# blyssprivacy/sdk

Hardware: AMD Instinct MI355X
Metric: PIR queries/sec (full answer path) on 2^20 items x 256 B (higher is better)
Workload: dtype u64; 1 GPU; spiral-rs process_query, c2 = {"db_item_size": 256, "instances": 1, "n": 2, "nu_1": 9, "nu_2": 11, "p": 256, "q2_bits": 20, "t_conv": 4, "t_exp_left": 8, "t_exp_right": 56, "t_gsw": 8}, encoded DB 64.0 GiB (56.0 GiB resident per GPU), unsharded, one query per step

## Files before the change

sdk_amd/csrc/bodies.hpp:

```cpp
#pragma once
#include "device_common.hpp"

namespace spiral {

__device__ __forceinline__ void ntt_fwd_body(const DevTables& T, const FwdDesc& d, int o, int c, u32* ldsA, u32* ldsB) {
  const int tau = threadIdx.x;
  const int rows = d.rdim * d.t;
  const int per_b = rows * d.cols;
  const int b = o / per_b;
  const int rem = o - b * per_b;
  const int row = rem / d.cols, col = rem - row * d.cols;
  const int kdig = row / d.rdim, j = row - kdig * d.rdim;
  long sb = d.src_idx ? (long)d.src_idx[b] : (long)b;
  if (d.delta_off) sb = (long)(b / d.delta_inner) * d.delta_outer_stride + (b % d.delta_inner);
  const u64* src = d.src + (sb * d.src_batch_stride + (long)(d.src_row0 + j) * d.src_cols + col) * N;
  const ModConst m = T.c.mod[c];
  const int sh = kdig * d.bits;
  const bool plain = (d.bits >= 64);
  const u64 mask = plain ? ~0ULL : ((1ULL << d.bits) - 1ULL);
  u32 v[8];
#pragma unroll
  for (int k = 0; k < 8; k++) {
    u64 x = src[tau + 256 * k];
    u64 piece = (sh >= 64) ? 0ULL : ((x >> sh) & mask);
// ... 45 lines not shown
  if (d.scal) {
    if (p >= d.n_polys) {
      const int e = p - d.n_polys;
      const int ct = d.scal_only_idx[e >> 1], r = e & 1;
      const long sp = ((long)(ct - d.scal_thresh) * 2 + r) * 2 * N, dp = ((long)ct * 2 + r) * 2 * N;
#pragma unroll
      for (int c = 0; c < 2; c++) {
        const uint4* a = reinterpret_cast<const uint4*>(d.src + sp + c * N + 8 * tau);
        const uint4* b = reinterpret_cast<const uint4*>(d.scal + c * N + 8 * tau);
        const uint4 a0 = a[0], a1 = a[1], b0 = b[0], b1 = b[1];
        const ModConst m = T.c.mod[c];
        uint4* o = reinterpret_cast<uint4*>(d.scal_dst + dp + c * N + 8 * tau);
        o[0] = make_uint4(reduce64((u64)a0.x * b0.x, m), reduce64((u64)a0.y * b0.y, m), reduce64((u64)a0.z * b0.z, m), reduce64((u64)a0.w * b0.w, m));
        o[1] = make_uint4(reduce64((u64)a1.x * b1.x, m), reduce64((u64)a1.y * b1.y, m), reduce64((u64)a1.z * b1.z, m), reduce64((u64)a1.w * b1.w, m));
      }
      return;
    }
    const int e = p / d.polys_per_idx, r = p - e * d.polys_per_idx;
    const int ct = d.idx[e];
    if (ct >= d.scal_thresh) {
      scal_store = base;
      base = (long)(ct - d.scal_thresh) * d.idx_stride + (long)r * d.poly_stride;
    }
  }
  u32 res[2][8];
#pragma unroll
  for (int c = 0; c < 2; c++) {
    const ModConst m = T.c.mod[c];
    const u32* src = d.src + base + (long)c * crt_stride;
    u32 v[8];
    if (z_stride == 1 && ((base | crt_stride | (scal_store < 0 ? 0 : scal_store)) & 3) == 0) {
      const uint4 a0 = reinterpret_cast<const uint4*>(src + 8 * tau)[0], a1 = reinterpret_cast<const uint4*>(src + 8 * tau)[1];
      v[0] = a0.x; v[1] = a0.y; v[2] = a0.z; v[3] = a0.w; v[4] = a1.x; v[5] = a1.y; v[6] = a1.z; v[7] = a1.w;
      if (d.premod) {
#pragma unroll
        for (int k = 0; k < 8; k++) v[k] %= m.q;
      }
      if (scal_store >= 0) {
        const uint4 s0 = reinterpret_cast<const uint4*>(d.scal + c * N + 8 * tau)[0], s1 = reinterpret_cast<const uint4*>(d.scal + c * N + 8 * tau)[1];
        const u32 sc[8] = {s0.x, s0.y, s0.z, s0.w, s1.x, s1.y, s1.z, s1.w};
#pragma unroll
        for (int k = 0; k < 8; k++) v[k] = reduce64((u64)v[k] * (u64)sc[k], m);
        uint4* o = reinterpret_cast<uint4*>(d.scal_dst + scal_store + (long)c * crt_stride + 8 * tau);
        o[0] = make_uint4(v[0], v[1], v[2], v[3]);
        o[1] = make_uint4(v[4], v[5], v[6], v[7]);
      }
// ... 216 lines not shown
```

sdk_amd/csrc/capi.cpp:

```cpp
#include <cstdlib>
#include <new>

#include "capi_internal.hpp"

using namespace spiral;

static thread_local std::string g_last_error;
static thread_local int g_last_rc = SP_OK;
static thread_local int g_shard_split_hint = 1;
int spiral::guarded_status(int rc, const char* what) {
  if (rc != SP_OK) g_last_error = what;
  g_last_rc = rc;
  return rc;
}
int spiral::null_handle_rc() { return g_last_rc != SP_OK ? g_last_rc : SP_E_ARG; }

void spiral::check_device(int dev) {
  int cur = 0;
  HIP_CHECK(hipGetDevice(&cur));
  if (cur != dev) throw ArgError("handle belongs to HIP device " + std::to_string(dev) + " but the current device is " + std::to_string(cur));
}

void spiral::download_ntt(Workspace& W, const u32* src, size_t words, uint64_t* host, DevBuf<u64>& tmp) {
  tmp.ensure(words);
// ... 611 lines not shown
  if (!name) return SP_E_ARG;
  set_tunable(name, value);
  return SP_OK;
}
extern "C" void sp_shard_split_hint_(int on) { g_shard_split_hint = on; }
extern "C" int sp_scatter_group_choice_(const sp_db_t* db, int G) {
  if (db && db->sparse) {
    tunables_new_call();
    return db->col_G == 1 && db->num_shards == G && sparse_group_min() != 0 ? SPARSE_GROUP_MAX : 1;
  }
  if (db && db->planar_resident) return db->num_shards == G && G > 1 ? planar_resident_group_max(db->nj) : 1;
  if (!db || !db->packed || db->col_G != 1 || db->num_shards != G) return 1;
  SweepBatchDesc d{};
  d.batch = SWEEP_BATCH_MAX;
  d.num_per = db->np_local;
  d.nj = db->nj;
  tunables_new_call();
  return sweep_batch_scatter_ok(d, G) && G <= (int)tunable("batch_scatter_max_g", BATCH_SCATTER_MAX_G_DEFAULT) ? SWEEP_BATCH_MAX : 1;
}
extern "C" int sp_shard_group_max_(const sp_db_t* db) {
  return db && db->planar_resident && db->num_shards > 1 ? planar_resident_group_max(db->nj) : SWEEP_BATCH_MAX;
}
extern "C" int sp_db_num_shards_(const sp_db_t* db) { return db ? db->num_shards : 0; }
void sp_set_last_error_(const char* msg) { g_last_error = msg ? msg : ""; }
void sp_note_path_(uint64_t bits) { note_path(bits); }

const char* sp_path_name(int bit) {
  static const char* names[] = {"sweep_packed_persist", "sweep_packed", "sweep_wide", "sweep_narrow", "sweep_batch",
                                "from_sweep4", "from_sweep1", "fold_fused", "fold_tail_delta", "fold_tail_literal",
                                "pipelined_fold_overlap", "expand_pruned", "pack_v1", "direct_upload", "scatter_out",
                                "from_sweep4_xcd_order", "fold_tail_persistent", "expand_round_one_launch", "sweep_sparse",
                                "rccl_in_library", "fold_wave", "cu_split_overlap", "expand_split", "pipe_class_split",
                                "sweep_batch_mfma", "custom_transport", "from_sweep_wave",
                                "fold_tail_batched", "sweep_ring", "sweep_batch_mfma_two_tiles", "fold_wave8", "sweep_batch_planar",
                                "expand_group", "expand_wave", "sweep_batch_scatter", "sparse_group_pass", "sweep_narrow_group"};
  return bit >= 0 && bit < (int)(sizeof(names) / sizeof(names[0])) ? names[bit] : nullptr;
}

int sp_device_count(void) {
  int n = 0;
  if (hipGetDeviceCount(&n) != hipSuccess) {
    (void)hipGetLastError();
    return 0;
  }
  return n;
}
// ... 811 lines not shown
```

sdk_amd/csrc/fold.hip:

```cpp
#include <type_traits>

#include "device_common.hpp"
#include "wave_ntt.hpp"
#include "bodies.hpp"

namespace spiral {

__device__ __forceinline__ bool fold_zero_shortcut(const u64* ct0, const u64* ct1, u64* out, int tau) {
  int nz0 = 0, nz1 = 0;
#pragma unroll
  for (int k = 0; k < 16; k++) {
    nz0 |= ct0[tau + 256 * k] != 0;
    nz1 |= ct1[tau + 256 * k] != 0;
  }
  const int any0 = __syncthreads_or(nz0), any1 = __syncthreads_or(nz1);
  if (any0 && any1) return false;
  const u64* src = any0 ? ct0 : ct1;
#pragma unroll
  for (int k = 0; k < 16; k++) out[tau + 256 * k] = src[tau + 256 * k];
  return true;
}

__global__ __launch_bounds__(256, 2) void k_fold_fused(DevTables T, FoldDesc d) {
  __shared__ u32 lds0[LDS_WORDS];
// ... 451 lines not shown

__global__ __launch_bounds__(256, 2) void k_expand_wave(DevTables T, ExpandWaveDesc d, GroupOff g) {
  extern __shared__ __attribute__((aligned(16))) u32 smem_fw[];
  u32* wbuf = smem_fw;
  u32* ltw = smem_fw + 4 * WBUF_WORDS;
  u64* raw0 = reinterpret_cast<u64*>(ltw + 2 * N);
  const int tau = threadIdx.x, lane = tau & 63;
  const int wv = __builtin_amdgcn_readfirstlane(tau >> 6);
  const int b = (int)blockIdx.x, c = (int)blockIdx.y, qi = (int)blockIdx.z;
  const ModConst m = T.c.mod[c];
  const u32* fw = T.tw + (size_t)c * 4 * N;
  const u64* src = group_rebase(d.raw, g.raw[qi]) + (size_t)d.pos[b] * 2 * N;
  const u32* A_w = group_rebase(d.A_w, g.pp[qi]);
  u32* vout = group_rebase(d.v, g.v[qi]);
  u32* mybuf = wbuf + wv * WBUF_WORDS;
  wtw_stage(ltw, wave_fwd_image(T.tw, c), tau);
#pragma unroll
  for (int k = 0; k < 8; k++) raw0[tau + 256 * k] = src[tau + 256 * k];
  __syncthreads();
  const u64 mask = (1ULL << d.bits) - 1ULL;
  u64 acc0[32], acc1[32];
#pragma unroll
  for (int k = 0; k < 32; k++) acc0[k] = acc1[k] = 0;
#pragma unroll 1
  for (int dg = wv; dg <= d.t; dg += 4) {
    int ln = lane;
    const u32* fwi = fw;
    asm volatile("" : "+v"(ln));
    asm volatile("" : "+s"(fwi));
    WaveScalarTw stw;
    wntt_scalar_tw(stw, fwi);
    u32 v[32];
    if (dg < d.t) {
      const int sh = dg * d.bits;
#pragma unroll
      for (int k = 0; k < 32; k++) v[k] = sh < 64 ? (u32)((raw0[64 * k + ln] >> (sh & 63)) & mask) : 0u;
    } else {
#pragma unroll
      for (int k = 0; k < 32; k++) v[k] = reduce64(src[(size_t)N + 64 * k + ln], m);
    }
    SP_SB();
    const u32* a0 = dg < d.t ? A_w + ((size_t)dg * 2 + c) * N : d.const_w;
    const u32* a1 = dg < d.t ? A_w + ((size_t)(d.t + dg) * 2 + c) * N : d.const_w + N;
    FoldMac hk{acc0, acc1, reinterpret_cast<const u32x4w_t*>(a0) + ln, reinterpret_cast<const u32x4w_t*>(a1) + ln};
    wntt_fwd<false>(v, ln, mybuf, fwi, stw, ltw, m.q, m.two_q, hk);
  }
  int lt = lane;
  asm volatile("" : "+v"(lt));
// ... 12 lines not shown
}
#define SP_ADD(R, REGION)                                                                              \
_Pragma("unroll") for (int g4 = 0; g4 < 8; g4++) {                                                   \
  const u32x4w_t t4 = sc[(REGION) * 512 + g4 * 64 + lt];                                             \
  R[4 * g4] = add_mod(R[4 * g4], t4.x, m.q); R[4 * g4 + 1] = add_mod(R[4 * g4 + 1], t4.y, m.q);      \
  R[4 * g4 + 2] = add_mod(R[4 * g4 + 2], t4.z, m.q); R[4 * g4 + 3] = add_mod(R[4 * g4 + 3], t4.w, m.q); \
}
  __syncthreads();
  if (wv == 2) { SP_PUT(r0, 0) SP_PUT(r1, 1) }
  if (wv == 3) { SP_PUT(r0, 2) SP_PUT(r1, 3) }
  __syncthreads();
  if (wv == 0) { SP_ADD(r0, 0) SP_ADD(r0, 2) }
  if (wv == 1) { SP_ADD(r1, 1) SP_ADD(r1, 3) }
  __syncthreads();
  if (wv == 0) { SP_PUT(r1, 0) }
  if (wv == 1) { SP_PUT(r0, 1) }
  __syncthreads();
  if (wv == 0) { SP_ADD(r0, 1) }
  if (wv == 1) { SP_ADD(r1, 0) }
#undef SP_PUT
#undef SP_ADD
  if (wv < 2) {
    u32* o = vout + ((size_t)d.out_idx[b] * 2 + c) * N + (size_t)wv * 2 * N + 32 * lt;
#pragma unroll
    for (int g4 = 0; g4 < 8; g4++) {
      const uint4 a = reinterpret_cast<const uint4*>(o)[g4];
      uint4 w;
      w.x = add_mod(wv == 0 ? r0[4 * g4] : r1[4 * g4], a.x, m.q);
      w.y = add_mod(wv == 0 ? r0[4 * g4 + 1] : r1[4 * g4 + 1], a.y, m.q);
      w.z = add_mod(wv == 0 ? r0[4 * g4 + 2] : r1[4 * g4 + 2], a.z, m.q);
      w.w = add_mod(wv == 0 ? r0[4 * g4 + 3] : r1[4 * g4 + 3], a.w, m.q);
      reinterpret_cast<uint4*>(o)[g4] = w;
    }
  }
}
void launch_expand_wave(const DevTables& T, const ExpandWaveDesc& d, const GroupOff& g, int B, hipStream_t s) {
  if (d.cnt <= 0 || B <= 0) return;
  const size_t lds = (size_t)(4 * WBUF_WORDS + 2 * N) * 4 + (size_t)N * 8;
  hipLaunchKernelGGL(k_expand_wave, dim3(d.cnt, 2, B), dim3(256), lds, s, T, d, g);
  launched(PATH_EXPAND_FUSED | PATH_EXPAND_WAVE, "k_expand_wave");
}

__global__ __launch_bounds__(256) void k_mats_to_wave(MatsToWaveDesc d) { mats_to_wave_body(d, blockIdx.x); }
void launch_mats_to_wave(u32* dst, const u32* src, size_t n_words, hipStream_t s, int half_polys) {
  if (n_words == 0) return;
  const MatsToWaveDesc d{dst, src, n_words, half_polys};
  hipLaunchKernelGGL(k_mats_to_wave, dim3((unsigned)((n_words + 255) / 256)), dim3(256), 0, s, d);
  launched(0, "k_mats_to_wave");
}
// ... 42 lines not shown
```

sdk_amd/csrc/kernels.hpp:

```cpp
#pragma once
#include <hip/hip_runtime.h>

#include <vector>

#include "params.hpp"

namespace spiral {

constexpr int N = (int)POLY_LEN;

struct DevTables {
  const u32* tw;
  DevConsts c;
};
__host__ __device__ inline const u32* inv_tables(const u32* tw, int c) { return tw + (size_t)8 * N + (size_t)c * 2 * N; }
__host__ __device__ inline const u32* wave_fwd_image(const u32* tw, int c) { return tw + (size_t)12 * N + (size_t)c * 2 * N; }
__host__ __device__ inline int wtw_phys(int idx) {
  if (idx >= 1024) {
    const int L = (idx - 1024) >> 4, r = (idx - 1024) & 15;
    return 1024 + 16 * L + 4 * (((r >> 2) + (L >> 2)) & 3) + (r & 3);
  }
  if (idx >= 512) {
    const int L = (idx - 512) >> 3, r = (idx - 512) & 7;
    return 512 + 8 * L + 4 * (((r >> 2) + (L >> 3)) & 1) + (r & 3);
// ... 61 lines not shown
};
void launch_ntt_fwd(const DevTables& T, const FwdDesc& d, hipStream_t s);
void launch_ntt_fwd3(const DevTables& T, const FwdDesc& d0, const FwdDesc& d1, const FwdDesc& d2, hipStream_t s);

float bench_ntt_core(const DevTables& T, int M, int blocks, int reps, u32* scratch, hipStream_t s);

struct InvDesc {
  const u32* src;
  const int* idx;
  int polys_per_idx;
  long idx_stride, poly_stride, crt_stride, z_stride;
  u64* dst;
  int n_polys;
  int premod;
  int sweep_np;
  int automorph_t;
  const u32* scal;
  u32* scal_dst;
  int scal_thresh;
  const int* scal_only_idx;
  int n_scalar_only;
  const u64* addend;
  int add_inner2, add_outer_stride;
};
void launch_ntt_inv(const DevTables& T, const InvDesc& d, hipStream_t s);
void launch_from_sweep4(const DevTables& T, const u32* src, int np, int n_planes, int premod, u64* dst, hipStream_t s);

struct MacDesc {
  const u32* A;
  const u32* B;
  u32* out;
  const u32* addend;
  const int* out_idx;
  int R, K;
  int A_row_stride;
  int batch_inner, batch_outer;
  long B_inner_stride, B_outer_stride;
  int split_k;
  long split_off;
  int out_batch_stride, out_row_stride;
  const u32* extra;
  const int* extra_idx;
  int extra_row;
};
void launch_mac(const DevTables& T, const MacDesc& d, hipStream_t s);
void launch_mac2(const DevTables& T, const MacDesc& d0, const MacDesc& d1, hipStream_t s);

struct ExpandSideDesc {
  const u64* raw;
  const int* pos;
  const int* out_idx;
  const u32* A;
  u32* v;
  int cnt, t, bits;
};
void launch_expand_round(const DevTables& T, const ExpandSideDesc& left, const ExpandSideDesc& right, hipStream_t s);
constexpr long EXPAND_ROUND_MIN_DEFAULT = 2048;

constexpr int GROUP_MAX = 16;
struct GroupOff {
  long long v[GROUP_MAX], raw[GROUP_MAX], dig[GROUP_MAX], ct1[GROUP_MAX], pp[GROUP_MAX];
};
void launch_ntt_inv_group(const DevTables& T, const InvDesc& d, const GroupOff& g, int B, hipStream_t s);
void launch_ntt_fwd3_group(const DevTables& T, const FwdDesc& d0, const FwdDesc& d1, const FwdDesc& d2, const GroupOff& g, int B,
                           hipStream_t s);
void launch_mac2_group(const DevTables& T, const MacDesc& d0, const MacDesc& d1, const GroupOff& g, int B, hipStream_t s);
void launch_expand_round_group(const DevTables& T, const ExpandSideDesc& left, const ExpandSideDesc& right, const GroupOff& g, int B,
                               hipStream_t s);
void launch_reorient_group(u64* out, const u32* v, int first, int step, int dim0, const GroupOff& g, int B, hipStream_t s);
void launch_copy_polys_group(u32* dst, const int* dst_idx, int dst_row_stride, const u32* src, const int* src_idx, int src_row_stride,
                             int R, int batch, const GroupOff& g, int B, hipStream_t s);
void launch_folding_neg_group(const DevTables& T, u32* mats, const u32* gadget_ntt, int nu2, int two_t, const GroupOff& g, int B,
                              hipStream_t s);
void launch_mats_to_wave_group(u32* dst, const u32* src, size_t n_words, int half_polys, const GroupOff& g, int B, hipStream_t s);
struct ExpandWaveDesc {
  const u64* raw;
  const int* pos;
  const int* out_idx;
  const u32* A_w;
  const u32* const_w;
  u32* v;
  int cnt, t, bits;
};
void launch_expand_wave(const DevTables& T, const ExpandWaveDesc& d, const GroupOff& g, int B, hipStream_t s);
constexpr long EXPAND_WAVE_MIN_DIGITS_DEFAULT = 16;
constexpr long EXPAND_GROUP_ROUND_MIN_DEFAULT = 4096;

struct FoldDesc {
  const u64* X;
  u64* Y;
  const u32* mats;
  int cur, half, planes;
  int t, bits;
  int t_live;
  int zero_shortcuts;
  const u32* mats_w;
};
void launch_mats_to_wave(u32* dst, const u32* src, size_t n_words, hipStream_t s, int half_polys = 0);
constexpr long FOLD_VARIANT_DEFAULT = 5;
void launch_fold_fused(const DevTables& T, const FoldDesc& d, hipStream_t s);

void launch_add_poly_into(const DevTables& T, u32* dst, const int* idx, const u32* src, int batch, hipStream_t s);
void launch_scalar_mul(const DevTables& T, u32* base, long dst_off, long src_off, const u32* scalar, int n_polys,
                       hipStream_t s);
void launch_add_polys_idx(const DevTables& T, u32* dst, const int* di, const u32* a, const int* ai, const u32* b,
// ... 249 lines not shown
```

sdk_amd/csrc/ntt.hip:

```cpp
#include "device_common.hpp"
#include "bodies.hpp"

namespace spiral {

template <int M>
__global__ __launch_bounds__(256) void k_ntt_core_bench(DevTables T, u32* out, int reps) {
  __shared__ u32 lds0[M * LDS_WORDS];
  __shared__ u32 lds1[M * LDS_WORDS];
  const int tau = threadIdx.x;
  const ModConst m = T.c.mod[blockIdx.x & 1];
  const u32* fw = T.tw + (size_t)(blockIdx.x & 1) * 4 * N;
  u32 v[M][8];
#pragma unroll
  for (int mm = 0; mm < M; mm++)
#pragma unroll
    for (int k = 0; k < 8; k++) v[mm][k] = (tau * 2654435761u + k * 40503u + mm + blockIdx.x) % m.q;
  u32* la = lds0;
  u32* lb = lds1;
  for (int r = 0; r < reps; r++) {
    const u32* fwk = fw;
    int tk = tau;
    asm volatile("" : "+s"(fwk));
    asm volatile("" : "+v"(tk));
    ntt_fwd_block_m<M>(v, tk, la, lb, fwk, fwk + N, m.q, m.two_q);
// ... 126 lines not shown
#pragma unroll
    for (int mm = 0; mm < GD; mm++) {
      const int kk = k0 + mm;
      if (kk < d.t) {
        const uint4* a0 = reinterpret_cast<const uint4*>(d.A + ((size_t)kk * 2 + c) * N + 8 * tk);
        const uint4* a1 = reinterpret_cast<const uint4*>(d.A + ((size_t)(d.t + kk) * 2 + c) * N + 8 * tk);
        const uint4 p0 = a0[0], p1 = a0[1], r0 = a1[0], r1 = a1[1];
        acc0[0] += (u64)p0.x * v[mm][0]; acc0[1] += (u64)p0.y * v[mm][1]; acc0[2] += (u64)p0.z * v[mm][2]; acc0[3] += (u64)p0.w * v[mm][3];
        acc0[4] += (u64)p1.x * v[mm][4]; acc0[5] += (u64)p1.y * v[mm][5]; acc0[6] += (u64)p1.z * v[mm][6]; acc0[7] += (u64)p1.w * v[mm][7];
        acc1[0] += (u64)r0.x * v[mm][0]; acc1[1] += (u64)r0.y * v[mm][1]; acc1[2] += (u64)r0.z * v[mm][2]; acc1[3] += (u64)r0.w * v[mm][3];
        acc1[4] += (u64)r1.x * v[mm][4]; acc1[5] += (u64)r1.y * v[mm][5]; acc1[6] += (u64)r1.z * v[mm][6]; acc1[7] += (u64)r1.w * v[mm][7];
      }
    }
    if (((k0 / GD) & 7) == 7) {
#pragma unroll
      for (int k = 0; k < 8; k++) {
        acc0[k] = reduce64(acc0[k], m);
        acc1[k] = reduce64(acc1[k], m);
      }
    }
    __syncthreads();
  }
  u32 e1[8];
#pragma unroll
  for (int k = 0; k < 8; k++) e1[k] = reduce64(src[(size_t)N + tau + 256 * k], m);
  ntt_fwd_block(e1, tau, lds0, lds1, fw, fw + N, m.q, m.two_q);
  u32* o0 = d.v + ((size_t)d.out_idx[b] * 2 + c) * N + 8 * tau;
  u32* o1 = o0 + (size_t)2 * N;
  const uint4 g0 = reinterpret_cast<const uint4*>(o0)[0], g1 = reinterpret_cast<const uint4*>(o0)[1];
  const uint4 h0 = reinterpret_cast<const uint4*>(o1)[0], h1 = reinterpret_cast<const uint4*>(o1)[1];
  const u32 ga[8] = {g0.x, g0.y, g0.z, g0.w, g1.x, g1.y, g1.z, g1.w};
  const u32 ha[8] = {h0.x, h0.y, h0.z, h0.w, h1.x, h1.y, h1.z, h1.w};
  u32 w0[8], w1[8];
#pragma unroll
  for (int k = 0; k < 8; k++) {
    w0[k] = reduce64(acc0[k] + ga[k], m);
    w1[k] = reduce64(acc1[k] + (u64)ha[k] + e1[k], m);
  }
  reinterpret_cast<uint4*>(o0)[0] = make_uint4(w0[0], w0[1], w0[2], w0[3]);
  reinterpret_cast<uint4*>(o0)[1] = make_uint4(w0[4], w0[5], w0[6], w0[7]);
  reinterpret_cast<uint4*>(o1)[0] = make_uint4(w1[0], w1[1], w1[2], w1[3]);
  reinterpret_cast<uint4*>(o1)[1] = make_uint4(w1[4], w1[5], w1[6], w1[7]);
}
__global__ __launch_bounds__(256) void k_expand_round(DevTables T, ExpandSideDesc dl, ExpandSideDesc dr) {
  __shared__ u32 lds0[EXPAND_GD * LDS_WORDS];
  __shared__ u32 lds1[EXPAND_GD * LDS_WORDS];
  const bool right = (int)blockIdx.x >= dl.cnt;
  expand_round_body(T, right ? dr : dl, (int)blockIdx.x - (right ? dl.cnt : 0), blockIdx.y, lds0, lds1);
}
__global__ __launch_bounds__(256) void k_expand_round_group(DevTables T, ExpandSideDesc dl, ExpandSideDesc dr, GroupOff g) {
  __shared__ u32 lds0[EXPAND_GD * LDS_WORDS];
  __shared__ u32 lds1[EXPAND_GD * LDS_WORDS];
  const int qi = blockIdx.z;
  const bool right = (int)blockIdx.x < dr.cnt;
  ExpandSideDesc d = right ? dr : dl;
  d.raw = group_rebase(d.raw, g.raw[qi]);
  d.A = group_rebase(d.A, g.pp[qi]);
  d.v = group_rebase(d.v, g.v[qi]);
  expand_round_body(T, d, (int)blockIdx.x - (right ? 0 : dr.cnt), blockIdx.y, lds0, lds1);
}
void launch_expand_round_group(const DevTables& T, const ExpandSideDesc& left, const ExpandSideDesc& right, const GroupOff& g, int B,
                               hipStream_t s) {
  const int total = std::max(left.cnt, 0) + std::max(right.cnt, 0);
  if (total <= 0 || B <= 0) return;
  ExpandSideDesc a = left, b = right;
  a.cnt = std::max(a.cnt, 0);
  b.cnt = std::max(b.cnt, 0);
  hipLaunchKernelGGL(k_expand_round_group, dim3(total, 2, B), dim3(256), 0, s, T, a, b, g);
  launched(PATH_EXPAND_FUSED | PATH_EXPAND_GROUP, "k_expand_round_group");
}
void launch_expand_round(const DevTables& T, const ExpandSideDesc& left, const ExpandSideDesc& right, hipStream_t s) {
  const int total = std::max(left.cnt, 0) + std::max(right.cnt, 0);
  if (total <= 0) return;
  ExpandSideDesc a = left, b = right;
  a.cnt = std::max(a.cnt, 0);
  b.cnt = std::max(b.cnt, 0);
  hipLaunchKernelGGL(k_expand_round, dim3(total, 2), dim3(256), 0, s, T, a, b);
  launched(PATH_EXPAND_FUSED, "k_expand_round");
}

__global__ __launch_bounds__(256) void k_ntt_inv(DevTables T, InvDesc d) {
  __shared__ u32 ldsA[LDS_WORDS];
  __shared__ u32 ldsB[LDS_WORDS];
  ntt_inv_body(T, d, blockIdx.x, ldsA, ldsB);
}
__global__ __launch_bounds__(256) void k_ntt_inv_group(DevTables T, InvDesc d, GroupOff g) {
  __shared__ u32 ldsA[LDS_WORDS];
  __shared__ u32 ldsB[LDS_WORDS];
  const int qi = blockIdx.y;
  d.src = group_rebase(d.src, g.v[qi]);
  d.scal_dst = group_rebase(d.scal_dst, g.v[qi]);
  d.dst = group_rebase(d.dst, g.raw[qi]);
  ntt_inv_body(T, d, blockIdx.x, ldsA, ldsB);
}
void launch_ntt_inv_group(const DevTables& T, const InvDesc& d, const GroupOff& g, int B, hipStream_t s) {
  const int blocks = d.n_polys + (d.scal ? 2 * d.n_scalar_only : 0);
  if (blocks <= 0 || B <= 0) return;
  hipLaunchKernelGGL(k_ntt_inv_group, dim3(blocks, B), dim3(256), 0, s, T, d, g);
  launched(PATH_EXPAND_GROUP, "k_ntt_inv_group");
}
void launch_ntt_inv(const DevTables& T, const InvDesc& d, hipStream_t s) {
  const int blocks = d.n_polys + (d.scal ? 2 * d.n_scalar_only : 0);
  if (blocks <= 0) return;
  hipLaunchKernelGGL(k_ntt_inv, dim3(blocks), dim3(256), 0, s, T, d);
  launched(d.sweep_np > 0 ? PATH_FROM_SWEEP1 : 0, "k_ntt_inv");
}

__global__ __launch_bounds__(256, 2) void k_from_sweep4(DevTables T, const u32* src, int np, int premod, u64* dst, int xcd_map) {
  __shared__ u32 lds0[4 * LDS_WORDS];
  __shared__ u32 lds1[4 * LDS_WORDS];
  const int tau = threadIdx.x;
  int g = blockIdx.x;
  if (xcd_map & 1) {
    const int xcd = g & 7, t = g >> 3;
    g = ((t >> 3) * 8 + xcd) * 8 + (t & 7);
// ... 64 lines not shown
```

sdk_amd/csrc/params.cpp:

```cpp
#include "params.hpp"
#include "kernels.hpp"

#include <cctype>
#include <cmath>
#include <map>
#include <stdexcept>

namespace spiral {

typedef unsigned __int128 u128;

u64 mul_mod(u64 a, u64 b, u64 m) { return (u64)((u128)a * b % m); }
u64 pow_mod(u64 a, u64 e, u64 m) {
  u64 r = 1 % m;
  a %= m;
  while (e) {
    if (e & 1) r = mul_mod(r, a, m);
    a = mul_mod(a, a, m);
    e >>= 1;
  }
  return r;
}
u64 inv_mod(u64 a, u64 m) {
  __int128 t = 0, nt = 1, r = m, nr = a % m;
// ... 102 lines not shown
      u64 half = (ipw & 1) ? (ipw + q) >> 1 : ipw >> 1;
      fw[idx] = (u32)pw;
      fwp[idx] = (u32)((pw << 32) / q);
      iw[idx] = (u32)half;
      iwp[idx] = (u32)((half << 32) / q);
      const u64 lz = idx < 2 ? mul_mod(ipw, n_inv, q) : ipw;
      lw[idx] = (u32)lz;
      lwp[idx] = (u32)((lz << 32) / q);
      pw = mul_mod(pw, psi, q);
      ipw = mul_mod(ipw, psi_inv, q);
    }
    if (poly_len == (size_t)N) {
      u32* img = ntt_tables.data() + (size_t)CRT_COUNT * 6 * poly_len + (size_t)c * 2 * poly_len;
      for (size_t i = 0; i < poly_len; i++) {
        const int ph = wtw_phys((int)i);
        img[ph] = 0u - fw[i];
        img[poly_len + ph] = fwp[i];
      }
    }
    dc.mod[c].q = (u32)q;
    dc.mod[c].two_q = (u32)(2 * q);
    dc.mod[c].m64 = (u64)((((u128)1) << 64) / q);
  }
  dc.Q = modulus;
  u64 inv = inv_mod(moduli[0] % moduli[1], moduli[1]);
  dc.q0_inv_q1 = (u32)inv;
  dc.q0_inv_q1_sh = (u32)((inv << 32) / moduli[1]);
}

static std::map<std::string, double> parse_flat_json(const std::string& s) {
  std::map<std::string, double> out;
  size_t i = 0, n = s.size();
  auto skip = [&]() {
    while (i < n && isspace((unsigned char)s[i])) i++;
  };
  skip();
  if (i >= n || s[i] != '{') throw std::runtime_error("params json: expected '{'");
  i++;
  for (;;) {
    skip();
    if (i < n && s[i] == '}') break;
    if (i >= n || (s[i] != '"' && s[i] != '\'')) throw std::runtime_error("params json: expected key");
    char qc = s[i++];
    size_t k0 = i;
    while (i < n && s[i] != qc) i++;
    if (i >= n) throw std::runtime_error("params json: unterminated key");
// ... 89 lines not shown
```

sdk_amd/csrc/params.hpp:

```cpp
#pragma once
static_assert(__BYTE_ORDER__ == __ORDER_LITTLE_ENDIAN__, "spiral_hip assumes a little-endian host");
#include <cstddef>
#include <cstdint>
#include <string>
#include <vector>

namespace spiral {

typedef uint64_t u64;
typedef uint32_t u32;

constexpr size_t POLY_LEN = 2048;
constexpr size_t POLY_LEN_LOG2 = 11;
constexpr size_t CRT_COUNT = 2;
constexpr u64 MODULUS_0 = 268369921ULL;
constexpr u64 MODULUS_1 = 249561089ULL;
constexpr size_t SEED_LENGTH = 32;

struct ModConst {
  u32 q;
  u32 two_q;
  u64 m64;
};

struct DevConsts {
  ModConst mod[2];
  u64 Q;
  u32 q0_inv_q1;
  u32 q0_inv_q1_sh;
};

struct Params {
  size_t poly_len = POLY_LEN, poly_len_log2 = POLY_LEN_LOG2, crt_count = CRT_COUNT;
  u64 moduli[2] = {MODULUS_0, MODULUS_1};
  u64 modulus = 0, modulus_log2 = 0;
  double noise_width = 6.4;
  size_t n = 0;
  u64 pt_modulus = 0, q2_bits = 0;
  size_t t_conv = 0, t_exp_left = 0, t_exp_right = 0, t_gsw = 0;
  bool expand_queries = true;
  size_t db_dim_1 = 0, db_dim_2 = 0, instances = 1, db_item_size = 0, version = 0;
  std::vector<u32> ntt_tables;
  DevConsts dc;

  size_t dim0() const { return (size_t)1 << db_dim_1; }
  size_t num_per() const { return (size_t)1 << db_dim_2; }
  size_t num_items() const { return dim0() * num_per(); }
  size_t trials() const { return n * n; }
  size_t planes() const { return instances * n * n; }
  size_t g() const;
  size_t stop_round() const;
  size_t setup_bytes() const;
  size_t query_bytes() const;
  size_t response_bytes() const;
  size_t db_words() const { return planes() * num_items() * poly_len; }
  bool has_expansion_right_on_wire() const { return version == 0 || t_exp_right != t_exp_left; }
  size_t bits_per(size_t dim) const;
  u64 q2() const;
  const u32* table(int crt, int which) const { return ntt_tables.data() + ((size_t)crt * 4 + which) * poly_len; }

  static Params from_json(const std::string& json);
  void finish();
};

u64 mul_mod(u64 a, u64 b, u64 m);
u64 pow_mod(u64 a, u64 e, u64 m);
// ... 4 lines not shown
```

sdk_amd/csrc/pipeline.hpp:

```cpp
#pragma once
#include <vector>

#include "server.hpp"

namespace spiral {

struct Workspace {
  const Params* P;
  DeviceState* D;
  int device = -1;
  hipStream_t stream = nullptr;
  hipStream_t stream2 = nullptr;
  std::vector<hipEvent_t> ev_plane;
  hipEvent_t ev_fold = nullptr;
  hipEvent_t ev_round0 = nullptr, ev_right = nullptr;
  bool right_pending = false;
  bool long_sweep_follows = false;
  hipEvent_t ev_sw[2] = {nullptr, nullptr};
  bool have_sweep_span = false;
  bool pipelined = false;
  hipEvent_t ev[5] = {nullptr, nullptr, nullptr, nullptr, nullptr};
  DevBuf<u64> q_raw;
  DevBuf<u32> v;
  DevBuf<u64> exp_raw;
// ... 19 lines not shown
  DevBuf<u64> group_q_raw;
  u64* h_packed = nullptr;
  size_t h_packed_words = 0;
  DevBuf<u64> enc_out;
  uint8_t* h_response = nullptr;
  bool host_pinned = true;
  int out_G = 1;
  bool zero_shortcuts = false;
  long fused_min_pairs = 256;

  Workspace(const Params& P, DeviceState& D);
  ~Workspace();
  Workspace(const Workspace&) = delete;
  Workspace& operator=(const Workspace&) = delete;
  void ensure_expand();
  void ensure_sweep();
  void ensure_finish();
  size_t plane_group() const;
};

void run_coefficient_expansion(Workspace& W, const sp_pp& pp, size_t g_rounds, const DeviceState::PrunedPlan* plan = nullptr,
                               int tree = 0, size_t r_begin = 0);
void join_right(Workspace& W);
void run_regev_to_gsw(Workspace& W, const sp_pp& pp, const u32* v_src, const int* src_ct, const int* src_poly);
void run_folding_neg(Workspace& W);
void run_mats_to_wave(Workspace& W, size_t levels, bool c_only = false);
void run_fold_operands(Workspace& W);
void run_begin_direct(Workspace& W, const uint8_t* query);
void run_begin_group(Workspace* const* Ws, const sp_pp* const* pps, const uint8_t* const* queries, const size_t* query_lens, int B);
void run_begin(Workspace& W, const sp_pp& pp, const uint8_t* query, size_t query_len, int j0 = 0, int nj = 0,
               const DeviceState::PrunedPlan* plan = nullptr);
void run_sweep_sparse(Workspace& W, const sp_db& db, const int* col_ptr, const int* col_rows, const int* col_slots);
void run_sweep_sparse_group(Workspace* const* Ws, int B, const sp_db& db, const int* col_ptr, const int* col_rows, const int* col_slots,
                            hipStream_t s);
void run_sweep_sparse_scatter(Workspace& W, const sp_db& db, const int* col_ptr, const int* col_rows, const int* col_slots, int G,
                              int plane0, int n_planes, bool per_plane);
void run_sweep_sparse_scatter_group(Workspace* const* Ws, int B, const sp_db& db, const int* col_ptr, const int* col_rows,
                                    const int* col_slots, int G, hipStream_t s);
std::unique_ptr<DeviceState::PrunedPlan> build_pruned_plan_rows(const Params& P, const std::vector<char>& rows);
void run_sweep(Workspace& W, const sp_db& db);
void run_sweep_pipelined(Workspace& W, const sp_db& db);
bool sweep_is_pipelined(const Params& p, const sp_db& db);
void launch_plane_sweep(Workspace& W, const sp_db& db, size_t plane);
bool fused_fold_supported(const Params& p);
struct FoldOpts {
  long fused_min_pairs;
// ... 16 lines not shown
```

sdk_amd/csrc/server.cpp:

```cpp
#include "server.hpp"

#include <algorithm>
#include <atomic>
#include <cstdlib>
#include <cstring>
#include <functional>

#include "pipeline.hpp"

namespace spiral {

void hip_check(hipError_t e, const char* what, const char* file, int line) {
  if (e != hipSuccess) {
    (void)hipGetLastError();
    throw HipError(std::string(what) + " failed at " + file + ":" + std::to_string(line) + ": " + hipGetErrorString(e));
  }
}

static std::mutex g_tun_mu;
static std::vector<std::pair<std::string, long>> g_tun;
static std::atomic<unsigned> g_tun_epoch{1};
static std::atomic<long> g_fresh_allocs{0};
void tunables_new_call() { g_tun_epoch.fetch_add(1, std::memory_order_relaxed); }
void set_tunable(const char* name, long v) {
// ... 343 lines not shown

std::unique_ptr<DeviceState::PrunedPlan> build_pruned_plan_rows(const Params& P, const std::vector<char>& rows) {
  auto pl = std::make_unique<DeviceState::PrunedPlan>();
  pl->j0 = -1;
  pl->nj = -1;
  std::vector<int> L;
  pl->rounds = build_round_plans(P, 0, 0, L, &rows);
  pl->rounds_even = build_round_plans(P, 0, 0, L, &rows, 1);
  pl->rounds_odd = build_round_plans(P, 0, 0, L, &rows, 2);
  pl->lists.alloc(std::max<size_t>(L.size(), 1));
  if (!L.empty()) upload_words(pl->lists.p, L.data(), L.size() * sizeof(int));
  return pl;
}

static std::unique_ptr<DeviceState> build_device_state(const Params& P, int device) {
  auto D = std::make_unique<DeviceState>();
  D->device = device;
  D->tw.alloc(P.ntt_tables.size());
  upload_words(D->tw.p, P.ntt_tables.data(), P.ntt_tables.size() * sizeof(u32));
  D->T.tw = D->tw.p;
  D->T.c = P.dc;
  const size_t g = P.expand_queries ? P.g() : 0;
  const size_t nu2 = P.db_dim_2;

  {
    std::vector<u64> raw(std::max<size_t>(g, 1) * POLY_LEN, 0);
    for (size_t r = 0; r < g && r < POLY_LEN_LOG2; r++) raw[r * POLY_LEN + (POLY_LEN - ((size_t)1 << r))] = P.modulus - 1;
    DevBuf<u64> d_raw(raw.size());
    h2d_sync(d_raw.p, raw.data(), raw.size() * 8);
    D->neg1.alloc(std::max<size_t>(g, 1) * 2 * POLY_LEN);
    FwdDesc f{d_raw.p, nullptr, D->neg1.p, (int)g, 1, 1, 1, 64, 1, 0, 1};
    launch_ntt_fwd(D->T, f, 0);
    HIP_CHECK(hipDeviceSynchronize());
  }
  {
    const size_t cols = 2 * P.t_gsw, bits = P.bits_per(P.t_gsw);
    std::vector<u64> raw(2 * cols * POLY_LEN, 0);
    for (size_t i = 0; i < 2; i++)
      for (size_t j = 0; j < P.t_gsw; j++) {
        if (bits * j >= 64) continue;
        raw[(i * cols + (i + j * 2)) * POLY_LEN] = 1ULL << (bits * j);
      }
    DevBuf<u64> d_raw(raw.size());
    h2d_sync(d_raw.p, raw.data(), raw.size() * 8);
    D->gadget_gsw.alloc(2 * cols * 2 * POLY_LEN);
    FwdDesc f{d_raw.p, nullptr, D->gadget_gsw.p, (int)(2 * cols), 1, 1, 1, 64, 1, 0, 1};
// ... 252 lines not shown
  const Params& p = *W.P;
  DeviceState& D = *W.D;
  u64* const exp_raw = tree == 2 ? W.exp_raw_r.p : W.exp_raw.p;
  u32* const exp_dig = tree == 2 ? W.exp_dig_r.p : W.exp_dig.p;
  u32* const exp_ct1 = tree == 2 ? W.exp_ct1_r.p : W.exp_ct1.p;
  const int tl = (int)p.t_exp_left, tr = (int)p.t_exp_right;
  RoundLaunches R{};
  InvDesc& inv = R.inv;
  inv.src = W.v.p;
  inv.idx = L + rp.all_ct;
  inv.polys_per_idx = 2;
  inv.idx_stride = 4 * POLY_LEN;
  inv.poly_stride = 2 * POLY_LEN;
  inv.crt_stride = POLY_LEN;
  inv.z_stride = 1;
  inv.dst = exp_raw;
  inv.n_polys = rp.n_all * 2;
  inv.automorph_t = rp.t_auto;
  inv.scal = D.neg1.p + r * 2 * POLY_LEN;
  inv.scal_dst = W.v.p;
  inv.scal_thresh = rp.num_in;
  inv.scal_only_idx = L + rp.skip2;
  inv.n_scalar_only = rp.n_skip2;
  for (int side = 0; side < 2; side++) {
    const int cnt = side == 0 ? rp.n_left : rp.n_right;
    const int t = side == 0 ? tl : tr;
    FwdDesc f{};
    f.src = exp_raw;
    f.src_idx = L + (side == 0 ? rp.left_pos : rp.right_pos);
    f.dst = exp_dig + (side == 0 ? 0 : (size_t)rp.n_left * tl * 2 * POLY_LEN);
    f.n_out = cnt * t;
    f.rdim = 1;
    f.cols = 1;
    f.t = t;
    f.bits = (int)p.bits_per(t);
    f.src_batch_stride = 2;
    f.src_row0 = 0;
    f.src_cols = 1;
    R.fd[side] = f;
  }
  {
    FwdDesc f1{};
    f1.src = exp_raw;
    f1.dst = exp_ct1;
    f1.n_out = rp.n_all;
    f1.rdim = 1;
    f1.cols = 1;
    f1.t = 1;
    f1.bits = 64;
    f1.src_batch_stride = 2;
    f1.src_row0 = 1;
    f1.src_cols = 1;
    R.fd[2] = f1;
  }
  R.round_transforms = (long)rp.n_left * tl + (long)rp.n_right * tr;
  R.digits_fit = R.fd[0].bits <= 28 && R.fd[1].bits <= 28;
  for (int side = 0; side < 2; side++) {
    const int cnt = side == 0 ? rp.n_left : rp.n_right;
    const int t = side == 0 ? tl : tr;
    const bool use_right = side == 1 && pp.has_right && p.db_dim_2 > 0;
    const size_t woff = use_right ? pp.off_right + r * 2 * tr : pp.off_left + r * 2 * tl;
    MacDesc m{};
    m.A = pp.all.p + woff * 2 * POLY_LEN;
    m.B = R.fd[side].dst;
    m.out = W.v.p;
    m.addend = W.v.p;
    m.out_idx = L + (side == 0 ? rp.left_out : rp.right_out);
    m.R = 2;
    m.K = t;
    m.batch_inner = cnt;
    m.batch_outer = 1;
    m.B_inner_stride = t;
    m.B_outer_stride = 0;
    m.split_k = t;
    m.split_off = 0;
    m.out_batch_stride = 0;
    m.out_row_stride = 1;
    m.extra = exp_ct1;
    m.extra_idx = L + (side == 0 ? rp.left_pos : rp.right_pos);
    m.extra_row = 1;
    R.md[side] = m;
    R.es[side] = ExpandSideDesc{R.fd[side].src, R.fd[side].src_idx, m.out_idx, m.A, m.out, m.batch_inner, R.fd[side].t, R.fd[side].bits};
  }
  return R;
}

void run_coefficient_expansion(Workspace& W, const sp_pp& pp, size_t g_rounds, const DeviceState::PrunedPlan* plan,
                               int tree, size_t r_begin) {
  DeviceState& D = *W.D;
  hipStream_t s = W.stream;
  const int* L = plan ? plan->lists.p : D.lists.p;
  const std::vector<RoundPlan>& rounds = tree == 1   ? (plan ? plan->rounds_even : D.rounds_even)
                                         : tree == 2 ? (plan ? plan->rounds_odd : D.rounds_odd)
                                                     : (plan ? plan->rounds : D.rounds);
  for (size_t r = r_begin; r < g_rounds; r++) {
    const RoundPlan& rp = rounds[r];
    if (rp.n_all == 0 && (tree != 0 || rp.n_skip2 == 0)) continue;
    const RoundLaunches R = round_launches(W, pp, rp, r, L, tree);
    const bool one_launch = R.round_transforms >= tunable("expand_round_min", EXPAND_ROUND_MIN_DEFAULT) && R.digits_fit &&
                            (tree != 2 || tunable("expand_round_odd", 0) != 0);
    launch_ntt_inv(D.T, R.inv, s);
    if (one_launch) {
      launch_expand_round(D.T, R.es[0], R.es[1], s);
    } else {
      launch_ntt_fwd3(D.T, R.fd[0], R.fd[1], R.fd[2], s);
// ... 28 lines not shown
  for (int i = 0; i < B; i++) {
    wave_ok = wave_ok && pps[i]->all_w.p != nullptr && pps[i]->all_w.n == pps[0]->all_w.n;
    if (wave_ok) gw.pp[i] = off(pps[i]->all_w.p, pps[0]->all_w.p);
  }
  for (size_t r = 0; r < g_rounds; r++) {
    const RoundPlan& rp = D.rounds[r];
    if (rp.n_all == 0 && rp.n_skip2 == 0) continue;
    const RoundLaunches R = round_launches(W0, *pps[0], rp, r, L, 0);
    launch_ntt_inv_group(D.T, R.inv, g, B, s);
    if (R.round_transforms * B >= group_min && R.digits_fit) {
      ExpandSideDesc coop[2] = {R.es[0], R.es[1]};
      for (int side = 1; side >= 0; side--)
        if (wave_ok && coop[side].cnt > 0 && coop[side].t >= wave_min_digits && coop[side].t <= 56) {
          ExpandWaveDesc w{};
          w.raw = coop[side].raw;
          w.pos = coop[side].pos;
          w.out_idx = coop[side].out_idx;
          w.A_w = pps[0]->all_w.p + (coop[side].A - pps[0]->all.p);
          w.const_w = pps[0]->all_w.p + pps[0]->all.n;
          w.v = coop[side].v;
          w.cnt = coop[side].cnt;
          w.t = coop[side].t;
          w.bits = coop[side].bits;
          launch_expand_wave(D.T, w, gw, B, s);
          coop[side].cnt = 0;
        }
      launch_expand_round_group(D.T, coop[0], coop[1], g, B, s);
    } else {
      launch_ntt_fwd3_group(D.T, R.fd[0], R.fd[1], R.fd[2], g, B, s);
      launch_mac2_group(D.T, R.md[0], R.md[1], g, B, s);
    }
  }
}

void run_regev_to_gsw(Workspace& W, const sp_pp& pp, const u32* v_src, const int* src_ct, const int* src_poly) {
  const Params& p = *W.P;
  DeviceState& D = *W.D;
  hipStream_t s = W.stream;
  const int* L = D.lists.p;
  const int nb = (int)(p.db_dim_2 * p.t_gsw);
  if (nb == 0) return;
  const int four_t = (int)(4 * p.t_gsw);
  launch_copy_polys(W.fold_mats.p, L + D.gsw_out_odd, four_t, v_src, src_poly, 1, 2, nb, s);
  InvDesc inv{};
  inv.src = v_src;
  inv.idx = src_ct;
// ... 254 lines not shown
}

void run_begin(Workspace& W, const sp_pp& pp, const uint8_t* query, size_t query_len, int j0, int nj,
               const DeviceState::PrunedPlan* plan) {
  const Params& p = *W.P;
  DeviceState& D = *W.D;
  if (query_len != p.query_bytes()) throw ArgError("query length " + std::to_string(query_len) + " != query_bytes " + std::to_string(p.query_bytes()));
  if (!p.expand_queries) {
    run_begin_direct(W, query);
    return;
  }
  run_begin_query_ct(W, query, query_len);
  hipStream_t s = W.stream;
  const size_t g = p.g();
  const bool prune = p.db_dim_2 > 0 && nj > 0 && (j0 != 0 || nj != (int)p.dim0());
  if (prune || (plan && p.db_dim_2 > 0)) note_path(PATH_EXPAND_PRUNED);
  const DeviceState::PrunedPlan* pl = plan && p.db_dim_2 > 0 ? plan : (prune ? &D.pruned_plan(p, j0, nj) : nullptr);
  const int* L = D.lists.p;
  const long split_mode = tunable("expand_split", -1);
  if (p.db_dim_2 > 0 && g >= 2 && (split_mode > 0 || (split_mode < 0 && W.long_sweep_follows))) {
    note_path(PATH_EXPAND_SPLIT);
    run_coefficient_expansion(W, pp, 1, pl, 0, 0);
    HIP_CHECK(hipEventRecord(W.ev_round0, s));
    HIP_CHECK(hipStreamWaitEvent(W.stream2, W.ev_round0, 0));
    on_stream(W, W.stream2, [&] {
      run_coefficient_expansion(W, pp, g, pl, 2, 1);
      run_regev_to_gsw(W, pp, W.v.p, L + D.gsw_src_ct, L + D.gsw_src_poly);
      run_fold_operands(W);
    });
    HIP_CHECK(hipEventRecord(W.ev_right, W.stream2));
    W.right_pending = true;
    run_coefficient_expansion(W, pp, g, pl, 1, 1);
    launch_reorient(W.qv.p, W.v.p, 0, 2, (int)p.dim0(), s);
    return;
  }
  run_coefficient_expansion(W, pp, g, pl);
  run_begin_after_rounds(W, pp);
}

void join_right(Workspace& W) {
  if (W.right_pending) HIP_CHECK(hipStreamWaitEvent(W.stream, W.ev_right, 0));
}

void run_sweep(Workspace& W, const sp_db& db) {
  if (db.planar_resident) throw ArgError("the single-query sweep kernels do not read a planar-resident database (sp_db_create_planar)");
  const Params& p = *W.P;
  W.ensure_sweep();
  SweepDesc d{db.words.p, W.qv.p, W.sweep_out.p, (int)p.planes(), db.np_local, (int)p.dim0(), db.j0, db.nj, db.packed, W.out_G};
  d.nt_store = (int)tunable("sweep_nt_store", 1);
  launch_sweep(W.D->T, d, W.stream);
}

void run_sweep_sparse(Workspace& W, const sp_db& db, const int* col_ptr, const int* col_rows, const int* col_slots) {
  const Params& p = *W.P;
  W.ensure_sweep();
  launch_sweep_sparse(W.D->T, col_ptr, col_rows, col_slots, db.polys.p, (int)p.planes(), W.v.p, 0,
// ... 520 lines not shown
```

sdk_amd/csrc/server.hpp:

```cpp
#pragma once
#include <cstdio>
#include <cstdlib>
#include <hip/hip_runtime.h>

#include <memory>
#include <mutex>
#include <stdexcept>
#include <string>
#include <unordered_map>
#include <vector>

#include "kernels.hpp"
#include "params.hpp"

namespace spiral {

struct HipError : std::runtime_error {
  explicit HipError(const std::string& s) : std::runtime_error(s) {}
};
struct ArgError : std::runtime_error {
  explicit ArgError(const std::string& s) : std::runtime_error(s) {}
};
struct OomError : std::runtime_error {
  explicit OomError(const std::string& s) : std::runtime_error(s) {}
// ... 60 lines not shown
void h2d_sync(void* dst, const void* host, size_t bytes);

void chacha20_keystream_u64(const uint8_t seed[32], u64* out, size_t count);

struct RoundPlan {
  int num_in = 0, t_auto = 0;
  int n_all = 0, n_left = 0, n_right = 0;
  size_t all_ct = 0;
  size_t all_row1 = 0;
  size_t left_pos = 0;
  size_t left_out = 0;
  size_t right_pos = 0, right_out = 0;
  size_t left_ct = 0, right_ct = 0;
  size_t skip2 = 0;
  int n_skip2 = 0;
};

struct DeviceState {
  int device = -1;
  DevTables T;
  DevBuf<u32> tw;
  DevBuf<u32> neg1;
  DevBuf<u32> gadget_gsw;
  DevBuf<int> lists;
  std::vector<RoundPlan> rounds;
  std::vector<RoundPlan> rounds_even, rounds_odd;
  size_t max_all = 0, max_left = 0, max_right = 0;
  struct PrunedPlan {
    int j0 = 0, nj = 0;
    std::vector<RoundPlan> rounds;
    std::vector<RoundPlan> rounds_even, rounds_odd;
    DevBuf<int> lists;
  };
  std::vector<std::unique_ptr<PrunedPlan>> pruned;
  std::mutex pruned_mu;
  const PrunedPlan& pruned_plan(const Params& P, int j0, int nj);
  size_t gsw_src_ct = 0;
  size_t gsw_src_poly = 0;
  size_t gsw_out_even = 0;
  size_t gsw_out_odd = 0;
  size_t pack_src_ct = 0;
  size_t pack_out = 0;
  size_t pack_row = 0;
  size_t v1_row1 = 0;
  size_t v1_shift_src = 0;
  size_t v1_rot_dst = 0, v1_rot_a = 0, v1_rot_b = 0;
// ... 81 lines not shown
```

Before: 92.77 queries/s.

## Apply automorphism to row-1 in NTT domain via permutation gather, skipping inverse/forward NTT

Precomputes, for each expansion round, the permutation the automorphism induces on NTT evaluation points. The inverse-NTT kernel then writes row 1 of odd ciphertexts straight into a gathered NTT-domain buffer instead of round-tripping it through an inverse transform, the automorphism and a forward transform. The expand and fold kernels read this buffer and skip the last gadget digit and the forward NTT for that row. A tunable to reorder the odd and even expansion sides is also added, with the default order unchanged. This adds host-side root computation, an extra device buffer and extra LDS synchronisation in the inverse body.

After: 92.96 queries/s (median of 5 runs). About the same (+0.2%).

```diff
diff --git a/sdk_amd/csrc/bodies.hpp b/sdk_amd/csrc/bodies.hpp
--- a/sdk_amd/csrc/bodies.hpp
+++ b/sdk_amd/csrc/bodies.hpp
@@ -91,6 +91,32 @@
       scal_store = base;
       base = (long)(ct - d.scal_thresh) * d.idx_stride + (long)r * d.poly_stride;
     }
+  }
+  if (d.row1_dst && d.idx && (p & 1)) {
+    const int e = p >> 1;
+    const uint4 j0 = reinterpret_cast<const uint4*>(d.row1_perm + 8 * tau)[0], j1 = reinterpret_cast<const uint4*>(d.row1_perm + 8 * tau)[1];
+#pragma unroll
+    for (int c = 0; c < 2; c++) {
+      const ModConst m = T.c.mod[c];
+      const u32* src = d.src + base + (long)c * crt_stride;
+      uint4 a0 = reinterpret_cast<const uint4*>(src + 8 * tau)[0], a1 = reinterpret_cast<const uint4*>(src + 8 * tau)[1];
+      if (scal_store >= 0) {
+        const uint4 s0 = reinterpret_cast<const uint4*>(d.scal + c * N + 8 * tau)[0], s1 = reinterpret_cast<const uint4*>(d.scal + c * N + 8 * tau)[1];
+        a0 = make_uint4(reduce64((u64)a0.x * s0.x, m), reduce64((u64)a0.y * s0.y, m), reduce64((u64)a0.z * s0.z, m), reduce64((u64)a0.w * s0.w, m));
+        a1 = make_uint4(reduce64((u64)a1.x * s1.x, m), reduce64((u64)a1.y * s1.y, m), reduce64((u64)a1.z * s1.z, m), reduce64((u64)a1.w * s1.w, m));
+        uint4* o = reinterpret_cast<uint4*>(d.scal_dst + scal_store + (long)c * crt_stride + 8 * tau);
+        o[0] = a0;
+        o[1] = a1;
+      }
+      if (c == 1) __syncthreads();
+      u32* l = ldsA + 8 * tau;
+      l[0] = a0.x; l[1] = a0.y; l[2] = a0.z; l[3] = a0.w; l[4] = a1.x; l[5] = a1.y; l[6] = a1.z; l[7] = a1.w;
+      __syncthreads();
+      uint4* o = reinterpret_cast<uint4*>(d.row1_dst + ((size_t)e * 2 + c) * N + 8 * tau);
+      o[0] = make_uint4(ldsA[j0.x], ldsA[j0.y], ldsA[j0.z], ldsA[j0.w]);
+      o[1] = make_uint4(ldsA[j1.x], ldsA[j1.y], ldsA[j1.z], ldsA[j1.w]);
+    }
+    return;
   }
   u32 res[2][8];
 #pragma unroll
diff --git a/sdk_amd/csrc/capi.cpp b/sdk_amd/csrc/capi.cpp
--- a/sdk_amd/csrc/capi.cpp
+++ b/sdk_amd/csrc/capi.cpp
@@ -657,6 +657,11 @@
   return db && db->planar_resident && db->num_shards > 1 ? planar_resident_group_max(db->nj) : SWEEP_BATCH_MAX;
 }
 extern "C" int sp_db_num_shards_(const sp_db_t* db) { return db ? db->num_shards : 0; }
+extern "C" int sp_row1_perm_(const sp_params_t* h, int round, int* out) {
+  if (!h || !out || round < 0 || (size_t)round >= h->p.poly_len_log2) return SP_E_ARG;
+  memcpy(out, h->p.row1_perm.data() + (size_t)round * h->p.poly_len, h->p.poly_len * sizeof(int));
+  return SP_OK;
+}
 void sp_set_last_error_(const char* msg) { g_last_error = msg ? msg : ""; }
 void sp_note_path_(uint64_t bits) { note_path(bits); }
 
diff --git a/sdk_amd/csrc/fold.hip b/sdk_amd/csrc/fold.hip
--- a/sdk_amd/csrc/fold.hip
+++ b/sdk_amd/csrc/fold.hip
@@ -497,8 +497,9 @@
   u64 acc0[32], acc1[32];
 #pragma unroll
   for (int k = 0; k < 32; k++) acc0[k] = acc1[k] = 0;
-#pragma unroll 1
-  for (int dg = wv; dg <= d.t; dg += 4) {
+  const int n_dig = d.ct1 ? d.t : d.t + 1;
+#pragma unroll 1
+  for (int dg = wv; dg < n_dig; dg += 4) {
     int ln = lane;
     const u32* fwi = fw;
     asm volatile("" : "+v"(ln));
@@ -557,9 +558,14 @@
 #undef SP_ADD
   if (wv < 2) {
     u32* o = vout + ((size_t)d.out_idx[b] * 2 + c) * N + (size_t)wv * 2 * N + 32 * lt;
+    const u32* e1 = wv == 1 && d.ct1 ? group_rebase(d.ct1, g.ct1[qi]) + ((size_t)d.pos[b] * 2 + c) * N + 32 * lt : nullptr;
 #pragma unroll
     for (int g4 = 0; g4 < 8; g4++) {
-      const uint4 a = reinterpret_cast<const uint4*>(o)[g4];
+      uint4 a = reinterpret_cast<const uint4*>(o)[g4];
+      if (e1) {
+        const uint4 x = reinterpret_cast<const uint4*>(e1)[g4];
+        a = make_uint4(add_mod(a.x, x.x, m.q), add_mod(a.y, x.y, m.q), add_mod(a.z, x.z, m.q), add_mod(a.w, x.w, m.q));
+      }
       uint4 w;
       w.x = add_mod(wv == 0 ? r0[4 * g4] : r1[4 * g4], a.x, m.q);
       w.y = add_mod(wv == 0 ? r0[4 * g4 + 1] : r1[4 * g4 + 1], a.y, m.q);
diff --git a/sdk_amd/csrc/kernels.hpp b/sdk_amd/csrc/kernels.hpp
--- a/sdk_amd/csrc/kernels.hpp
+++ b/sdk_amd/csrc/kernels.hpp
@@ -107,6 +107,8 @@
   int n_scalar_only;
   const u64* addend;
   int add_inner2, add_outer_stride;
+  const int* row1_perm;
+  u32* row1_dst;
 };
 void launch_ntt_inv(const DevTables& T, const InvDesc& d, hipStream_t s);
 void launch_from_sweep4(const DevTables& T, const u32* src, int np, int n_planes, int premod, u64* dst, hipStream_t s);
@@ -138,6 +140,7 @@
   const u32* A;
   u32* v;
   int cnt, t, bits;
+  const u32* ct1;
 };
 void launch_expand_round(const DevTables& T, const ExpandSideDesc& left, const ExpandSideDesc& right, hipStream_t s);
 constexpr long EXPAND_ROUND_MIN_DEFAULT = 2048;
@@ -166,6 +169,7 @@
   const u32* const_w;
   u32* v;
   int cnt, t, bits;
+  const u32* ct1;
 };
 void launch_expand_wave(const DevTables& T, const ExpandWaveDesc& d, const GroupOff& g, int B, hipStream_t s);
 constexpr long EXPAND_WAVE_MIN_DIGITS_DEFAULT = 16;
diff --git a/sdk_amd/csrc/ntt.hip b/sdk_amd/csrc/ntt.hip
--- a/sdk_amd/csrc/ntt.hip
+++ b/sdk_amd/csrc/ntt.hip
@@ -172,9 +172,15 @@
     __syncthreads();
   }
   u32 e1[8];
-#pragma unroll
-  for (int k = 0; k < 8; k++) e1[k] = reduce64(src[(size_t)N + tau + 256 * k], m);
-  ntt_fwd_block(e1, tau, lds0, lds1, fw, fw + N, m.q, m.two_q);
+  if (d.ct1) {
+    const uint4* s1 = reinterpret_cast<const uint4*>(d.ct1 + ((size_t)d.pos[b] * 2 + c) * N + 8 * tau);
+    const uint4 c0 = s1[0], c1 = s1[1];
+    e1[0] = c0.x; e1[1] = c0.y; e1[2] = c0.z; e1[3] = c0.w; e1[4] = c1.x; e1[5] = c1.y; e1[6] = c1.z; e1[7] = c1.w;
+  } else {
+#pragma unroll
+    for (int k = 0; k < 8; k++) e1[k] = reduce64(src[(size_t)N + tau + 256 * k], m);
+    ntt_fwd_block(e1, tau, lds0, lds1, fw, fw + N, m.q, m.two_q);
+  }
   u32* o0 = d.v + ((size_t)d.out_idx[b] * 2 + c) * N + 8 * tau;
   u32* o1 = o0 + (size_t)2 * N;
   const uint4 g0 = reinterpret_cast<const uint4*>(o0)[0], g1 = reinterpret_cast<const uint4*>(o0)[1];
@@ -207,6 +213,7 @@
   d.raw = group_rebase(d.raw, g.raw[qi]);
   d.A = group_rebase(d.A, g.pp[qi]);
   d.v = group_rebase(d.v, g.v[qi]);
+  if (d.ct1) d.ct1 = group_rebase(d.ct1, g.ct1[qi]);
   expand_round_body(T, d, (int)blockIdx.x - (right ? 0 : dr.cnt), blockIdx.y, lds0, lds1);
 }
 void launch_expand_round_group(const DevTables& T, const ExpandSideDesc& left, const ExpandSideDesc& right, const GroupOff& g, int B,
@@ -241,6 +248,7 @@
   d.src = group_rebase(d.src, g.v[qi]);
   d.scal_dst = group_rebase(d.scal_dst, g.v[qi]);
   d.dst = group_rebase(d.dst, g.raw[qi]);
+  if (d.row1_dst) d.row1_dst = group_rebase(d.row1_dst, g.ct1[qi]);
   ntt_inv_body(T, d, blockIdx.x, ldsA, ldsB);
 }
 void launch_ntt_inv_group(const DevTables& T, const InvDesc& d, const GroupOff& g, int B, hipStream_t s) {
diff --git a/sdk_amd/csrc/params.cpp b/sdk_amd/csrc/params.cpp
--- a/sdk_amd/csrc/params.cpp
+++ b/sdk_amd/csrc/params.cpp
@@ -148,6 +148,33 @@
     dc.mod[c].two_q = (u32)(2 * q);
     dc.mod[c].m64 = (u64)((((u128)1) << 64) / q);
   }
+  row1_perm.assign(poly_len_log2 * poly_len, 0);
+  for (int c = 0; c < 2; c++) {
+    const u64 q = moduli[c];
+    const u32* fw = table(c, 0);
+    std::vector<u64> root(poly_len, 0);
+    root[1] = 1;
+    for (size_t mm = 1, t = poly_len / 2; mm < poly_len; mm <<= 1, t >>= 1)
+      for (size_t i = 0; i < mm; i++)
+        for (size_t j = 2 * i * t; j < 2 * i * t + t; j++) {
+          const u64 x = root[j], y = mul_mod(root[j + t], fw[mm + i], q);
+          root[j] = (x + y) % q;
+          root[j + t] = (x + q - y) % q;
+        }
+    std::map<u64, int> at;
+    for (size_t j = 0; j < poly_len; j++) at[root[j]] = (int)j;
+    if (at.size() != poly_len) throw std::runtime_error("transform roots are not distinct");
+    for (size_t r = 0; r < poly_len_log2; r++) {
+      const u64 t_auto = (poly_len >> r) + 1;
+      for (size_t j = 0; j < poly_len; j++) {
+        const auto it = at.find(pow_mod(root[j], t_auto, q));
+        if (it == at.end()) throw std::runtime_error("automorphism leaves the transform's roots");
+        int& slot = row1_perm[r * poly_len + j];
+        if (c == 1 && slot != it->second) throw std::runtime_error("the two moduli order their roots differently");
+        slot = it->second;
+      }
+    }
+  }
   dc.Q = modulus;
   u64 inv = inv_mod(moduli[0] % moduli[1], moduli[1]);
   dc.q0_inv_q1 = (u32)inv;
diff --git a/sdk_amd/csrc/params.hpp b/sdk_amd/csrc/params.hpp
--- a/sdk_amd/csrc/params.hpp
+++ b/sdk_amd/csrc/params.hpp
@@ -42,6 +42,7 @@
   size_t db_dim_1 = 0, db_dim_2 = 0, instances = 1, db_item_size = 0, version = 0;
   std::vector<u32> ntt_tables;
   DevConsts dc;
+  std::vector<int> row1_perm;
 
   size_t dim0() const { return (size_t)1 << db_dim_1; }
   size_t num_per() const { return (size_t)1 << db_dim_2; }
diff --git a/sdk_amd/csrc/pipeline.hpp b/sdk_amd/csrc/pipeline.hpp
--- a/sdk_amd/csrc/pipeline.hpp
+++ b/sdk_amd/csrc/pipeline.hpp
@@ -65,6 +65,7 @@
 void run_coefficient_expansion(Workspace& W, const sp_pp& pp, size_t g_rounds, const DeviceState::PrunedPlan* plan = nullptr,
                                int tree = 0, size_t r_begin = 0);
 void join_right(Workspace& W);
+constexpr long EXPAND_ORDER_DEFAULT = 0;
 void run_regev_to_gsw(Workspace& W, const sp_pp& pp, const u32* v_src, const int* src_ct, const int* src_poly);
 void run_folding_neg(Workspace& W);
 void run_mats_to_wave(Workspace& W, size_t levels, bool c_only = false);
diff --git a/sdk_amd/csrc/server.cpp b/sdk_amd/csrc/server.cpp
--- a/sdk_amd/csrc/server.cpp
+++ b/sdk_amd/csrc/server.cpp
@@ -389,6 +389,8 @@
   D->T.c = P.dc;
   const size_t g = P.expand_queries ? P.g() : 0;
   const size_t nu2 = P.db_dim_2;
+  D->row1_perm.alloc(P.row1_perm.size());
+  upload_words(D->row1_perm.p, P.row1_perm.data(), P.row1_perm.size() * sizeof(int));
 
   {
     std::vector<u64> raw(std::max<size_t>(g, 1) * POLY_LEN, 0);
@@ -687,6 +689,11 @@
   inv.scal_thresh = rp.num_in;
   inv.scal_only_idx = L + rp.skip2;
   inv.n_scalar_only = rp.n_skip2;
+  const bool gather = tunable("expand_row1_gather", 1) != 0 && r < POLY_LEN_LOG2;
+  if (gather) {
+    inv.row1_perm = D.row1_perm.p + r * POLY_LEN;
+    inv.row1_dst = exp_ct1;
+  }
   for (int side = 0; side < 2; side++) {
     const int cnt = side == 0 ? rp.n_left : rp.n_right;
     const int t = side == 0 ? tl : tr;
@@ -716,6 +723,7 @@
     f1.src_batch_stride = 2;
     f1.src_row0 = 1;
     f1.src_cols = 1;
+    if (gather) f1.n_out = 0;
     R.fd[2] = f1;
   }
   R.round_transforms = (long)rp.n_left * tl + (long)rp.n_right * tr;
@@ -745,7 +753,8 @@
     m.extra_idx = L + (side == 0 ? rp.left_pos : rp.right_pos);
     m.extra_row = 1;
     R.md[side] = m;
-    R.es[side] = ExpandSideDesc{R.fd[side].src, R.fd[side].src_idx, m.out_idx, m.A, m.out, m.batch_inner, R.fd[side].t, R.fd[side].bits};
+    R.es[side] = ExpandSideDesc{R.fd[side].src, R.fd[side].src_idx, m.out_idx, m.A, m.out, m.batch_inner, R.fd[side].t, R.fd[side].bits,
+                                gather ? exp_ct1 : nullptr};
   }
   return R;
 }
@@ -820,6 +829,7 @@
           w.cnt = coop[side].cnt;
           w.t = coop[side].t;
           w.bits = coop[side].bits;
+          w.ct1 = coop[side].ct1;
           launch_expand_wave(D.T, w, gw, B, s);
           coop[side].cnt = 0;
         }
@@ -1120,16 +1130,21 @@
     note_path(PATH_EXPAND_SPLIT);
     run_coefficient_expansion(W, pp, 1, pl, 0, 0);
     HIP_CHECK(hipEventRecord(W.ev_round0, s));
-    HIP_CHECK(hipStreamWaitEvent(W.stream2, W.ev_round0, 0));
-    on_stream(W, W.stream2, [&] {
-      run_coefficient_expansion(W, pp, g, pl, 2, 1);
-      run_regev_to_gsw(W, pp, W.v.p, L + D.gsw_src_ct, L + D.gsw_src_poly);
-      run_fold_operands(W);
-    });
-    HIP_CHECK(hipEventRecord(W.ev_right, W.stream2));
-    W.right_pending = true;
+    const bool odd_first = tunable("expand_order", EXPAND_ORDER_DEFAULT) <= 0;
+    auto odd_side = [&] {
+      HIP_CHECK(hipStreamWaitEvent(W.stream2, W.ev_round0, 0));
+      on_stream(W, W.stream2, [&] {
+        run_coefficient_expansion(W, pp, g, pl, 2, 1);
+        run_regev_to_gsw(W, pp, W.v.p, L + D.gsw_src_ct, L + D.gsw_src_poly);
+        run_fold_operands(W);
+      });
+      HIP_CHECK(hipEventRecord(W.ev_right, W.stream2));
+      W.right_pending = true;
+    };
+    if (odd_first) odd_side();
     run_coefficient_expansion(W, pp, g, pl, 1, 1);
     launch_reorient(W.qv.p, W.v.p, 0, 2, (int)p.dim0(), s);
+    if (!odd_first) odd_side();
     return;
   }
   run_coefficient_expansion(W, pp, g, pl);
diff --git a/sdk_amd/csrc/server.hpp b/sdk_amd/csrc/server.hpp
--- a/sdk_amd/csrc/server.hpp
+++ b/sdk_amd/csrc/server.hpp
@@ -106,6 +106,7 @@
   DevBuf<u32> tw;
   DevBuf<u32> neg1;
   DevBuf<u32> gadget_gsw;
+  DevBuf<int> row1_perm;
   DevBuf<int> lists;
   std::vector<RoundPlan> rounds;
   std::vector<RoundPlan> rounds_even, rounds_odd;
```
